# PaddlePaddle/PaddleRobotics

Measured on NVIDIA H100. Metric: env-steps/sec (A1, 4096 envs), higher is better.
Workload: dtype f32

## Files before the change

paddlerobotics_b200/csrc/b2q_math.cuh:

```cuda
#pragma once
#include <cmath>
#include <cstdint>

#if defined(__CUDACC__)
#define B2Q_HD __host__ __device__ __forceinline__
#define B2Q_D __device__ __forceinline__
#else
#define B2Q_HD inline
#define B2Q_D inline
#endif

namespace b2q {

B2Q_HD float m_sqrt(float x) { return sqrtf(x); }
B2Q_HD double m_sqrt(double x) { return sqrt(x); }
#if defined(__CUDA_ARCH__)
B2Q_HD float m_rsqrt(float x) { return rsqrtf(x); }
#else
B2Q_HD float m_rsqrt(float x) { return 1.0f / sqrtf(x); }
#endif
B2Q_HD double m_rsqrt(double x) { return 1.0 / sqrt(x); }
B2Q_HD float m_sin(float x) { return sinf(x); }
B2Q_HD double m_sin(double x) { return sin(x); }
B2Q_HD float m_cos(float x) { return cosf(x); }
// ... 15 lines not shown
B2Q_HD float m_min(float a, float b) { return fminf(a, b); }
B2Q_HD double m_min(double a, double b) { return fmin(a, b); }
B2Q_HD float m_max(float a, float b) { return fmaxf(a, b); }
B2Q_HD double m_max(double a, double b) { return fmax(a, b); }
B2Q_HD float m_fma(float a, float b, float c) { return fmaf(a, b, c); }
B2Q_HD double m_fma(double a, double b, double c) { return fma(a, b, c); }
B2Q_HD bool m_isfinite(float x) { return (x - x) == 0.0f; }
B2Q_HD bool m_isfinite(double x) { return (x - x) == 0.0; }
B2Q_HD bool m_isnan(float x) { return x != x; }
B2Q_HD bool m_isnan(double x) { return x != x; }

B2Q_HD float m_log(float x) { return logf(x); }
B2Q_HD double m_log(double x) { return log(x); }

B2Q_HD uint32_t mulhi32(uint32_t a, uint32_t b) { return (uint32_t)(((uint64_t)a * (uint64_t)b) >> 32); }
B2Q_HD void philox4(uint64_t seed, uint32_t c0, uint32_t c1, uint32_t c2, uint32_t out[4]) {
  uint32_t c3 = 0, k0 = (uint32_t)seed, k1 = (uint32_t)(seed >> 32);
  for (int i = 0; i < 10; i++) {
    uint32_t h0 = mulhi32(0xD2511F53u, c0), l0 = 0xD2511F53u * c0, h1 = mulhi32(0xCD9E8D57u, c2), l1 = 0xCD9E8D57u * c2;
    uint32_t n0 = h1 ^ c1 ^ k0, n2 = h0 ^ c3 ^ k1;
    c0 = n0; c1 = l1; c2 = n2; c3 = l0;
    k0 += 0x9E3779B9u; k1 += 0xBB67AE85u;
  }
  out[0] = c0; out[1] = c1; out[2] = c2; out[3] = c3;
}
template <typename T> B2Q_HD void philox_normal4(uint64_t seed, uint32_t c0, uint32_t c1, uint32_t c2, T n[4]) {
  uint32_t r[4]; philox4(seed, c0, c1, c2, r);
  const T two_pi = T(6.283185307179586476925286766559), sc = T(1.0 / 16777216.0);
  T u0 = (T(r[0] >> 8) + T(0.5)) * sc, u1 = (T(r[1] >> 8) + T(0.5)) * sc, u2 = (T(r[2] >> 8) + T(0.5)) * sc, u3 = (T(r[3] >> 8) + T(0.5)) * sc;
  T ra = m_sqrt(T(-2) * m_log(u0)), rb = m_sqrt(T(-2) * m_log(u2));
  n[0] = ra * m_cos(two_pi * u1); n[1] = ra * m_sin(two_pi * u1); n[2] = rb * m_cos(two_pi * u3); n[3] = rb * m_sin(two_pi * u3);
}

#if defined(__CUDA_ARCH__)
B2Q_HD float m_rcp(float x) { float r; asm("rcp.approx.ftz.f32 %0, %1;" : "=f"(r) : "f"(x)); return fmaf(r, fmaf(-x, r, 1.0f), r); }
#else
B2Q_HD float m_rcp(float x) { return 1.0f / x; }
#endif
B2Q_HD double m_rcp(double x) { return 1.0 / x; }

B2Q_HD void m_sincos(float a, float& s, float& c) {
  float q = rintf(a * 0.636619772367581343f);
  int n = (int)q;
  float r = fmaf(q, -1.57079601287841796875f, a);
  r = fmaf(q, -3.1391647326017846353352069854736328125e-7f, r);
  r = fmaf(q, -5.390302529957764765543e-15f, r);
  float r2 = r * r;
  float sp = fmaf(fmaf(fmaf(-1.95152959e-4f, r2, 8.33216087e-3f), r2, -1.66666546e-1f), r2 * r, r);
  float cp = fmaf(fmaf(fmaf(fmaf(2.44331571e-5f, r2, -1.38873163e-3f), r2, 4.16666457e-2f), r2, -0.5f), r2, 1.0f);
  float ss = (n & 1) ? cp : sp, cc = (n & 1) ? sp : cp;
  s = (n & 2) ? -ss : ss;
  c = ((n + 1) & 2) ? -cc : cc;
}
B2Q_HD void m_sincos(double a, double& s, double& c) { s = sin(a); c = cos(a); }

template <typename T>
struct V3 {
  T x, y, z;
};
template <typename T> B2Q_HD V3<T> mk(T x, T y, T z) { V3<T> r; r.x = x; r.y = y; r.z = z; return r; }
template <typename T> B2Q_HD V3<T> operator+(V3<T> a, V3<T> b) { return mk<T>(a.x + b.x, a.y + b.y, a.z + b.z); }
template <typename T> B2Q_HD V3<T> operator-(V3<T> a, V3<T> b) { return mk<T>(a.x - b.x, a.y - b.y, a.z - b.z); }
template <typename T> B2Q_HD V3<T> operator-(V3<T> a) { return mk<T>(-a.x, -a.y, -a.z); }
template <typename T> B2Q_HD V3<T> operator*(V3<T> a, T s) { return mk<T>(a.x * s, a.y * s, a.z * s); }
template <typename T> B2Q_HD V3<T> operator*(T s, V3<T> a) { return mk<T>(a.x * s, a.y * s, a.z * s); }
template <typename T> B2Q_HD T dot(V3<T> a, V3<T> b) { return a.x * b.x + a.y * b.y + a.z * b.z; }
// ... 1 lines not shown

template <typename T>
struct S3 {
  T xx, xy, xz, yy, yz, zz;
};
template <typename T> B2Q_HD V3<T> mul(const S3<T>& s, V3<T> v) {
  return mk<T>(s.xx * v.x + s.xy * v.y + s.xz * v.z, s.xy * v.x + s.yy * v.y + s.yz * v.z, s.xz * v.x + s.yz * v.y + s.zz * v.z);
}
template <typename T> B2Q_HD S3<T> operator+(const S3<T>& a, const S3<T>& b) { S3<T> r = {a.xx + b.xx, a.xy + b.xy, a.xz + b.xz, a.yy + b.yy, a.yz + b.yz, a.zz + b.zz}; return r; }
template <typename T> B2Q_HD S3<T> point_inertia(T m, V3<T> c) {
  S3<T> r = {m * (c.y * c.y + c.z * c.z), -m * c.x * c.y, -m * c.x * c.z, m * (c.x * c.x + c.z * c.z), -m * c.y * c.z, m * (c.x * c.x + c.y * c.y)};
  return r;
}

template <typename T>
struct R3 {
  V3<T> cx, cy, cz;
};
template <typename T> B2Q_HD V3<T> rot(const R3<T>& R, V3<T> v) { return R.cx * v.x + R.cy * v.y + R.cz * v.z; }
template <typename T> B2Q_HD V3<T> rotT(const R3<T>& R, V3<T> v) { return mk<T>(dot(R.cx, v), dot(R.cy, v), dot(R.cz, v)); }
template <typename T> B2Q_HD S3<T> rot_sym(const R3<T>& R, const S3<T>& I) {
  V3<T> a = R.cx * I.xx + R.cy * I.xy + R.cz * I.xz;
  V3<T> b = R.cx * I.xy + R.cy * I.yy + R.cz * I.yz;
  V3<T> c = R.cx * I.xz + R.cy * I.yz + R.cz * I.zz;
  S3<T> o;
  o.xx = a.x * R.cx.x + b.x * R.cy.x + c.x * R.cz.x;
  o.xy = a.x * R.cx.y + b.x * R.cy.y + c.x * R.cz.y;
  o.xz = a.x * R.cx.z + b.x * R.cy.z + c.x * R.cz.z;
  o.yy = a.y * R.cx.y + b.y * R.cy.y + c.y * R.cz.y;
  o.yz = a.y * R.cx.z + b.y * R.cy.z + c.y * R.cz.z;
  o.zz = a.z * R.cx.z + b.z * R.cy.z + c.z * R.cz.z;
  return o;
}
template <typename T> B2Q_HD R3<T> quat_to_R(T x, T y, T z, T w) {
  R3<T> R;
  R.cx = mk<T>(1 - 2 * (y * y + z * z), 2 * (x * y + z * w), 2 * (x * z - y * w));
  R.cy = mk<T>(2 * (x * y - z * w), 1 - 2 * (x * x + z * z), 2 * (y * z + x * w));
  R.cz = mk<T>(2 * (x * z + y * w), 2 * (y * z - x * w), 1 - 2 * (x * x + y * y));
  return R;
}
template <typename T> B2Q_HD V3<T> quat_to_rpy(T x, T y, T z, T w) {
  T s = 2 * (w * y - z * x);
  s = m_min(m_max(s, T(-1)), T(1));
  return mk<T>(m_atan2(2 * (w * x + y * z), 1 - 2 * (x * x + y * y)), m_asin(s), m_atan2(2 * (w * z + x * y), 1 - 2 * (y * y + z * z)));
}

template <typename T>
struct V6 {
  V3<T> a, l;
};
template <typename T> B2Q_HD V6<T> operator+(V6<T> p, V6<T> q) { V6<T> r; r.a = p.a + q.a; r.l = p.l + q.l; return r; }
template <typename T> B2Q_HD V6<T> operator-(V6<T> p, V6<T> q) { V6<T> r; r.a = p.a - q.a; r.l = p.l - q.l; return r; }
template <typename T> B2Q_HD V6<T> operator*(V6<T> p, T s) { V6<T> r; r.a = p.a * s; r.l = p.l * s; return r; }
template <typename T> B2Q_HD T dot6(V6<T> p, V6<T> q) { return dot(p.a, q.a) + dot(p.l, q.l); }
template <typename T> B2Q_HD T get6(const V6<T>& v, int i) { return i == 0 ? v.a.x : i == 1 ? v.a.y : i == 2 ? v.a.z : i == 3 ? v.l.x : i == 4 ? v.l.y : v.l.z; }

B2Q_HD constexpr int tri(int i, int j) { return i >= j ? i * (i + 1) / 2 + j : j * (j + 1) / 2 + i; }

template <typename T> B2Q_HD void chol6(T* S , T* Li ) {
#pragma unroll
  for (int j = 0; j < 6; j++) {
    T d = S[tri(j, j)];
#pragma unroll
    for (int k = 0; k < j; k++) d -= S[tri(j, k)] * S[tri(j, k)];
    T inv = m_rsqrt(d);
    S[tri(j, j)] = d * inv;
// ... 33 lines not shown
```

paddlerobotics_b200/csrc/b2q_sim.cuh:

```cuda
#pragma once
#include "b2q_math.cuh"

namespace b2q {

constexpr int NS = 37;
constexpr int NP = 15;
constexpr int NE = 16;
constexpr int OBS_DIM = 49;
constexpr int INFO_DIM = 56;
constexpr int ETG_H = 20;

template <typename T>
struct alignas(4 * sizeof(T)) P4 {
  T x, y, z, w;
};

template <typename T>
struct LegModel {
  T p1[3];
  T lhip;
  T com[3][3];
  T I[3][6];
  T m[3];
};
// ... 10 lines not shown
  T knee_r;
  int obs_dim, obs_identity;
  int obs_src[OBS_DIM];
  T obs_scale[OBS_DIM], obs_shift[OBS_DIM];
};
template <typename T>
struct Cfg {
  T dt; int R; int iters; T erp, warm, margin; int interp; T tau_limit; int settle_steps;
  int filter; T fb0, fb1, fb2, fa1, fa2; int etg; int max_steps;
  T etg_T, etg_T2, etg_sigma_sq, etg_amp, etg_ph0, etg_ph1;
  T w_torso, w_feet, w_up, w_tau, w_stand, w_badfoot, w_footcontact, w_done, reward_p, vel_d;
  int terrain, hf_nx, hf_ny; T hf_x0, hf_y0, hf_cell, hf_icell, idt; const T* hf;
  int clip_cmd; T max_dq;
  int noise_on; T noise[5]; unsigned long long noise_seed;
  int stuck, body_coll;
  int motor_mode, jlim, extf, knee; T damp[4];
};
constexpr int STUCK_H = 10;
template <typename T>
struct Buffers {
  int N, Dm;
  P4<T>* state;
  P4<T>* snap;
  P4<T>* snap_obs;
  const P4<T>* param;
  const P4<T>* etg;
  P4<T>* ring;
  int* step_count;
  P4<T>* pos_hist;
  const P4<T>* extf;
};
template <typename T>
struct LaneParam {
  T kp[3], kd[3], iscale[3], mscale[3], m0s, I0s[3], mu, latency;
  V3<T> g;
};
template <typename T>
struct LaneState {
  V3<T> pos; T qx, qy, qz, qw; V3<T> vlin, vang;
  T q[3], qd[3]; T lam_n; int contact;
  T lam_lim[3];
};

template <typename T> B2Q_HD void sincos_t(T a, T& s, T& c) { m_sincos(a, s, c); }

template <typename T>
B2Q_HD T terrain_height(const Cfg<T>& cf, T x, T y, V3<T>& n) {
  if (cf.terrain == 0) { n = mk<T>(0, 0, 1); return T(0); }
  T fx = (x - cf.hf_x0) * cf.hf_icell, fy = (y - cf.hf_y0) * cf.hf_icell;
  fx = m_min(m_max(fx, T(0)), T(cf.hf_nx) - T(1.000001));
  fy = m_min(m_max(fy, T(0)), T(cf.hf_ny) - T(1.000001));
  int ix = (int)fx, iy = (int)fy;
  if (ix > cf.hf_nx - 2) ix = cf.hf_nx - 2;
  if (iy > cf.hf_ny - 2) iy = cf.hf_ny - 2;
  T tx = fx - T(ix), ty = fy - T(iy);
  const T* h = cf.hf; int nx = cf.hf_nx;
  T h00 = h[iy * nx + ix], h10 = h[iy * nx + ix + 1], h01 = h[(iy + 1) * nx + ix], h11 = h[(iy + 1) * nx + ix + 1];
  T hh = (1 - tx) * (1 - ty) * h00 + tx * (1 - ty) * h10 + (1 - tx) * ty * h01 + tx * ty * h11;
  T dhdx = ((1 - ty) * (h10 - h00) + ty * (h11 - h01)) * cf.hf_icell;
  T dhdy = ((1 - tx) * (h01 - h00) + tx * (h11 - h10)) * cf.hf_icell;
  T inv = m_rsqrt(dhdx * dhdx + dhdy * dhdy + T(1));
  n = mk<T>(-dhdx * inv, -dhdy * inv, inv);
  return hh;
}

template <typename T>
struct LegKin {
// ... 110 lines not shown
    for (int i = 0; i < n; i++) {
      T ln = lam[i] + (vec[idx[i] * 4 + 1] - uu[i]) / W[i * NRW + i];
      if (par[i] >= 0) { T lim = mu * lam[par[i]]; ln = m_min(m_max(ln, -lim), lim); } else ln = m_max(ln, T(0));
      T dl = ln - lam[i]; lam[i] = ln;
      for (int j = 0; j < n; j++) uu[j] += W[j * NRW + i] * dl;
    }
  }
  for (int e = 0; e < RPL; e++) { const int q = pos_of[RPL * k + e]; lk[e] = q >= 0 ? lam[q] : T(0); }
  cm.sync();
}

template <typename T, int FEAT, class Comm>
B2Q_HD void substep(const Comm& cm, const Cfg<T>& cf, const Model<T>& md, const LaneParam<T>& pr, LaneState<T>& s,
                    const T* target, T* tau_out, V3<T> fext = V3<T>{0, 0, 0}, const T* hyb = nullptr ) {
  const int k = cm.leg();
  const LegModel<T>& lm = md.leg[k];
  const T dt = cf.dt, idt = cf.idt;
  R3<T> R = quat_to_R(s.qx, s.qy, s.qz, s.qw);
  V3<T> wB = rotT(R, s.vang), vB = rotT(R, s.vlin), gB = rotT(R, pr.g);

  T tau[3];
#pragma unroll
  for (int j = 0; j < 3; j++) {
    T cmd = target[j];
    if (cf.clip_cmd) cmd = m_min(m_max(cmd, s.q[j] - cf.max_dq), s.q[j] + cf.max_dq);
    T t = T(-1) * (pr.kp[j] * (s.q[j] - cmd)) - pr.kd[j] * (s.qd[j] - T(0));
    if (FEAT && cf.motor_mode == 1) t = target[j];
    if (FEAT && cf.motor_mode == 2) t = T(-1) * (hyb[j] * (s.q[j] - cmd)) - hyb[6 + j] * (s.qd[j] - hyb[3 + j]) + hyb[9 + j];
    if (cf.tau_limit > T(0)) t = m_min(m_max(t, -cf.tau_limit), cf.tau_limit);
    tau[j] = t; tau_out[j] = t;
  }

  LegKin<T> K; leg_kin(md, lm, s.q, K);
  const V3<T> a1 = mk<T>(1, 0, 0), a2 = K.a2;
  V3<T> cL[3]; S3<T> IL[3]; T mL[3];
  {
    const R3<T>* Rs[3] = {&K.R1, &K.R2, &K.R3m};
    const V3<T> ps[3] = {K.p1, K.p2, K.p3};
#pragma unroll
    for (int i = 0; i < 3; i++) {
      cL[i] = ps[i] + rot(*Rs[i], mk<T>(lm.com[i][0], lm.com[i][1], lm.com[i][2]));
      S3<T> Il = {lm.I[i][0], lm.I[i][1], lm.I[i][2], lm.I[i][3], lm.I[i][4], lm.I[i][5]};
      S3<T> Ib = rot_sym(*Rs[i], Il);
      T sc = pr.iscale[i];
      IL[i].xx = Ib.xx * sc; IL[i].xy = Ib.xy * sc; IL[i].xz = Ib.xz * sc; IL[i].yy = Ib.yy * sc; IL[i].yz = Ib.yz * sc; IL[i].zz = Ib.zz * sc;
      mL[i] = lm.m[i] * pr.mscale[i];
    }
  }
  V3<T> w1 = wB + a1 * s.qd[0], w2 = w1 + a2 * s.qd[1], w3 = w2 + a2 * s.qd[2];
  V3<T> pdd0 = cross(wB, vB) - gB;
  V3<T> al1 = cross(wB, a1) * s.qd[0];
  V3<T> pdd1 = pdd0 + cross(wB, cross(wB, K.p1));
  V3<T> al2 = al1 + cross(w1, a2) * s.qd[1];
  V3<T> d21 = K.p2 - K.p1;
  V3<T> pdd2 = pdd1 + cross(al1, d21) + cross(w1, cross(w1, d21));
  V3<T> al3 = al2 + cross(w2, a2) * s.qd[2];
  V3<T> d32 = K.p3 - K.p2;
  V3<T> pdd3 = pdd2 + cross(al2, d32) + cross(w2, cross(w2, d32));
  V3<T> fL[3], nL[3];
  {
    const V3<T> ws[3] = {w1, w2, w3}, als[3] = {al1, al2, al3}, pdds[3] = {pdd1, pdd2, pdd3}, ps[3] = {K.p1, K.p2, K.p3};
#pragma unroll
    for (int i = 0; i < 3; i++) {
      V3<T> r = cL[i] - ps[i];
      V3<T> cdd = pdds[i] + cross(als[i], r) + cross(ws[i], cross(ws[i], r));
      fL[i] = cdd * mL[i];
      nL[i] = mul(IL[i], als[i]) + cross(ws[i], mul(IL[i], ws[i]));
    }
  }
  V3<T> F3 = fL[2], N3 = nL[2] + cross(cL[2] - K.p3, fL[2]);
  V3<T> F2 = fL[1] + F3, N2 = nL[1] + cross(cL[1] - K.p2, fL[1]) + N3 + cross(d32, F3);
  V3<T> F1 = fL[0] + F2, N1 = nL[0] + cross(cL[0] - K.p1, fL[0]) + N2 + cross(d21, F2);
  T hj[3] = {dot(a1, N1), dot(a2, N2), dot(a2, N3)};
  V3<T> NO = N1 + cross(K.p1, F1);

  T m3c = mL[2], m2c = mL[1] + m3c, m1c = mL[0] + m2c;
  V3<T> h3c = cL[2] * mL[2], h2c = cL[1] * mL[1] + h3c, h1c = cL[0] * mL[0] + h2c;
  S3<T> I3c = IL[2] + point_inertia(mL[2], cL[2]);
  S3<T> I2c = IL[1] + point_inertia(mL[1], cL[1]) + I3c;
  S3<T> I1c = IL[0] + point_inertia(mL[0], cL[0]) + I2c;
  V3<T> v1 = cross(K.p1, a1), v2 = cross(K.p2, a2), v3 = cross(K.p3, a2);
  V6<T> Fc[3];
  Fc[0].a = mul(I1c, a1) + cross(h1c, v1); Fc[0].l = v1 * m1c + cross(a1, h1c);
  Fc[1].a = mul(I2c, a2) + cross(h2c, v2); Fc[1].l = v2 * m2c + cross(a2, h2c);
  Fc[2].a = mul(I3c, a2) + cross(h3c, v3); Fc[2].l = v3 * m3c + cross(a2, h3c);
  T M11 = dot(a1, Fc[0].a) + dot(v1, Fc[0].l);
  T M21 = dot(a1, Fc[1].a) + dot(v1, Fc[1].l), M22 = dot(a2, Fc[1].a) + dot(v2, Fc[1].l);
  T M31 = dot(a1, Fc[2].a) + dot(v1, Fc[2].l), M32 = dot(a2, Fc[2].a) + dot(v2, Fc[2].l), M33 = dot(a2, Fc[2].a) + dot(v3, Fc[2].l);
  T D[3][3];
  {
    T c00 = M22 * M33 - M32 * M32, c01 = M31 * M32 - M21 * M33, c02 = M21 * M32 - M31 * M22;
    T det = M11 * c00 + M21 * c01 + M31 * c02, id = m_rcp(det);
    D[0][0] = c00 * id; D[0][1] = D[1][0] = c01 * id; D[0][2] = D[2][0] = c02 * id;
    D[1][1] = (M11 * M33 - M31 * M31) * id; D[1][2] = D[2][1] = (M31 * M21 - M11 * M32) * id;
    D[2][2] = (M11 * M22 - M21 * M21) * id;
  }
  T bj[3] = {tau[0] - hj[0], tau[1] - hj[1], tau[2] - hj[2]};
  T Fa[3][6], FD[3][6];
#pragma unroll
  for (int i = 0; i < 3; i++) v6_to_arr(Fc[i], Fa[i]);
#pragma unroll
  for (int j = 0; j < 3; j++) {
#pragma unroll
    for (int c = 0; c < 6; c++) FD[j][c] = m_fma(Fa[2][c], D[2][j], m_fma(Fa[1][c], D[1][j], Fa[0][c] * D[0][j]));
  }

  T S[21], r6[6];
  {
    const T Z = T(0);
    const T Cf[6][6] = {{I1c.xx, I1c.xy, I1c.xz, Z, -h1c.z, h1c.y},
                        {I1c.xy, I1c.yy, I1c.yz, h1c.z, Z, -h1c.x},
                        {I1c.xz, I1c.yz, I1c.zz, -h1c.y, h1c.x, Z},
                        {Z, h1c.z, -h1c.y, m1c, Z, Z},
                        {-h1c.z, Z, h1c.x, Z, m1c, Z},
                        {h1c.y, -h1c.x, Z, Z, Z, m1c}};
#pragma unroll
    for (int i = 0; i < 6; i++) {
#pragma unroll
      for (int j = 0; j <= i; j++) {
        T v = Cf[i][j];
#pragma unroll
        for (int k = 0; k < 3; k++) v = m_fma(Fa[k][j], -FD[k][i], v);
        S[tri(i, j)] = cm.sum4(v);
      }
    }
    const T NOa[6] = {NO.x, NO.y, NO.z, F1.x, F1.y, F1.z};
#pragma unroll
    for (int i = 0; i < 6; i++) {
      T v = -NOa[i];
#pragma unroll
      for (int k = 0; k < 3; k++) v = m_fma(FD[k][i], -bj[k], v);
      r6[i] = cm.sum4(v);
    }
  }
  {
    T sx = m_sqrt(pr.I0s[0]), sy = m_sqrt(pr.I0s[1]), sz = m_sqrt(pr.I0s[2]);
    S3<T> I0 = {md.I0[0] * sx * sx, md.I0[1] * sx * sy, md.I0[2] * sx * sz, md.I0[3] * sy * sy, md.I0[4] * sy * sz, md.I0[5] * sz * sz};
    T m0 = md.m0 * pr.m0s;
    S[tri(0, 0)] += I0.xx; S[tri(1, 0)] += I0.xy; S[tri(1, 1)] += I0.yy; S[tri(2, 0)] += I0.xz; S[tri(2, 1)] += I0.yz; S[tri(2, 2)] += I0.zz;
    S[tri(3, 3)] += m0; S[tri(4, 4)] += m0; S[tri(5, 5)] += m0;
    V3<T> n0 = cross(wB, mul(I0, wB)), f0 = pdd0 * m0;
    if (FEAT) {
      T lv = m_sqrt(dot(vB, vB)), lw = m_sqrt(dot(wB, wB));
      f0 = f0 + vB * (m0 * (cf.damp[0] + cf.damp[1] * lv));
      n0 = n0 + mul(I0, wB) * (cf.damp[2] + cf.damp[3] * lw);
      if (cf.extf) f0 = f0 - rotT(R, fext);
    }
    r6[0] -= n0.x; r6[1] -= n0.y; r6[2] -= n0.z; r6[3] -= f0.x; r6[4] -= f0.y; r6[5] -= f0.z;
  }
  T Li[6];
  chol6(S, Li);
  fwd6(S, Li, r6); bwd6(S, Li, r6);
  V6<T> nud = arr_to_v6(r6);
  T qdd[3];
  {
    T t[3] = {bj[0] - dot6(Fc[0], nud), bj[1] - dot6(Fc[1], nud), bj[2] - dot6(Fc[2], nud)};
#pragma unroll
    for (int j = 0; j < 3; j++) qdd[j] = D[j][0] * t[0] + D[j][1] * t[1] + D[j][2] * t[2];
  }
  V3<T> wBs = wB + nud.a * dt, vBs = vB + (nud.l + cross(wB, vB)) * dt;
  T qds[3] = {s.qd[0] + dt * qdd[0], s.qd[1] + dt * qdd[1], s.qd[2] + dt * qdd[2]};

  V3<T> toe_w = s.pos + rot(R, K.toe), n_w;
  T hgt = terrain_height(cf, toe_w.x, toe_w.y, n_w);
  T dist = toe_w.z - hgt - md.foot_r;
  bool act = dist < cf.margin;
  V3<T> t1w = mk<T>(1 - n_w.x * n_w.x, -n_w.x * n_w.y, -n_w.x * n_w.z);
  t1w = t1w * m_rsqrt(dot(t1w, t1w));
  V3<T> t2w = cross(n_w, t1w);
  V3<T> eB[3] = {rotT(R, n_w), rotT(R, t1w), rotT(R, t2w)};
  V3<T> xc = K.toe - eB[0] * md.foot_r;
  T Jk[3][3], u[3], Y[3][6], Wl[3][3];
  {
    V3<T> r1 = cross(a1, xc - K.p1), r2 = cross(a2, xc - K.p2), r3 = cross(a2, xc - K.p3);
#pragma unroll
    for (int e = 0; e < 3; e++) {
      Jk[e][0] = dot(eB[e], r1); Jk[e][1] = dot(eB[e], r2); Jk[e][2] = dot(eB[e], r3);
      V6<T> Jb; Jb.a = cross(xc, eB[e]); Jb.l = eB[e];
      u[e] = dot(Jb.a, wBs) + dot(Jb.l, vBs) + Jk[e][0] * qds[0] + Jk[e][1] * qds[1] + Jk[e][2] * qds[2];
      const T Jba[6] = {Jb.a.x, Jb.a.y, Jb.a.z, Jb.l.x, Jb.l.y, Jb.l.z};
#pragma unroll
      for (int c = 0; c < 6; c++) {
        T g = Jba[c];
#pragma unroll
        for (int j = 0; j < 3; j++) g = m_fma(FD[j][c], -Jk[e][j], g);
        Y[e][c] = g;
      }
      fwd6(S, Li, Y[e]);
    }
#pragma unroll
    for (int e = 0; e < 3; e++) {
      T dj[3];
#pragma unroll
      for (int i = 0; i < 3; i++) dj[i] = D[i][0] * Jk[e][0] + D[i][1] * Jk[e][1] + D[i][2] * Jk[e][2];
#pragma unroll
      for (int e2 = 0; e2 < 3; e2++) Wl[e2][e] = Jk[e2][0] * dj[0] + Jk[e2][1] * dj[1] + Jk[e2][2] * dj[2];
    }
  }
  T lk[3] = {T(0), T(0), T(0)};
  T lkx[6] = {T(0), T(0), T(0), T(0), T(0), T(0)}, Yx[6][6], Jx[6][3];
#pragma unroll
  for (int e = 0; e < 6; e++) {
#pragma unroll
    for (int c = 0; c < 6; c++) Yx[e][c] = T(0);
    Jx[e][0] = Jx[e][1] = Jx[e][2] = T(0);
  }
  bool general = false;
  if constexpr (FEAT != 0) {
    bool need = false;
    T kdist = T(1); V3<T> kn_w = mk<T>(0, 0, 1);
    if (cf.jlim) {
#pragma unroll
      for (int j = 0; j < 3; j++) need = need || (s.q[j] - md.qlo[j] < JLIM_GAP) || (md.qhi[j] - s.q[j] < JLIM_GAP);
    }
    if (cf.knee) {
      V3<T> kw = s.pos + rot(R, K.p3);
      kdist = kw.z - terrain_height(cf, kw.x, kw.y, kn_w) - md.knee_r;
      need = need || (kdist < cf.margin);
    }
    if ((cf.jlim || cf.knee) && cm.any(need)) {
      T Y9[RPL][6], u9[RPL], targ9[RPL], warm9[RPL], blk[45], Jall[RPL][3]; bool act9[RPL];
#pragma unroll
      for (int e = 0; e < 3; e++) {
#pragma unroll
        for (int c = 0; c < 6; c++) Y9[e][c] = Y[e][c];
        u9[e] = u[e]; targ9[e] = T(0); warm9[e] = T(0); act9[e] = act;
        Jall[e][0] = Jk[e][0]; Jall[e][1] = Jk[e][1]; Jall[e][2] = Jk[e][2];
      }
      targ9[0] = dist > T(0) ? -dist * idt : cf.erp * (-dist) * idt; warm9[0] = cf.warm * s.lam_n;
      {
        const bool kact = cf.knee && (kdist < cf.margin);
        V3<T> t1k = mk<T>(1 - kn_w.x * kn_w.x, -kn_w.x * kn_w.y, -kn_w.x * kn_w.z);
        t1k = t1k * m_rsqrt(dot(t1k, t1k));
        V3<T> t2k = cross(kn_w, t1k);
        V3<T> ek[3] = {rotT(R, kn_w), rotT(R, t1k), rotT(R, t2k)};
        V3<T> xk = K.p3 - ek[0] * md.knee_r;
        V3<T> r1 = cross(a1, xk - K.p1), r2 = cross(a2, xk - K.p2), r3 = cross(a2, xk - K.p3);
#pragma unroll
        for (int e = 0; e < 3; e++) {
          T jr[3] = {dot(ek[e], r1), dot(ek[e], r2), dot(ek[e], r3)};
          V6<T> Jb; Jb.a = cross(xk, ek[e]); Jb.l = ek[e];
          u9[3 + e] = dot(Jb.a, wBs) + dot(Jb.l, vBs) + jr[0] * qds[0] + jr[1] * qds[1] + jr[2] * qds[2];
#pragma unroll
          for (int i = 0; i < 6; i++) Yx[e][i] = get6(Jb, i) - (FD[0][i] * jr[0] + FD[1][i] * jr[1] + FD[2][i] * jr[2]);
          fwd6(S, Li, Yx[e]);
          Jx[e][0] = jr[0]; Jx[e][1] = jr[1]; Jx[e][2] = jr[2];
          targ9[3 + e] = T(0); warm9[3 + e] = T(0); act9[3 + e] = kact;
        }
        targ9[3] = kdist > T(0) ? -kdist * idt : cf.erp * (-kdist) * idt;
      }
#pragma unroll
      for (int j = 0; j < 3; j++) {
        T glo = s.q[j] - md.qlo[j], ghi = md.qhi[j] - s.q[j], gap = glo, sj = T(1);
        if (ghi < glo) { gap = ghi; sj = T(-1); }
#pragma unroll
        for (int i = 0; i < 6; i++) Yx[3 + j][i] = -sj * FD[j][i];
        fwd6(S, Li, Yx[3 + j]);
        Jx[3 + j][0] = j == 0 ? sj : T(0); Jx[3 + j][1] = j == 1 ? sj : T(0); Jx[3 + j][2] = j == 2 ? sj : T(0);
        u9[6 + j] = sj * qds[j];
        targ9[6 + j] = gap > T(0) ? -gap * idt : cf.erp * (-gap) * idt;
        warm9[6 + j] = cf.warm * s.lam_lim[j];
        act9[6 + j] = cf.jlim && (gap < JLIM_GAP);
      }
#pragma unroll
      for (int e = 0; e < 6; e++) {
#pragma unroll
        for (int c = 0; c < 6; c++) Y9[3 + e][c] = Yx[e][c];
        Jall[3 + e][0] = Jx[e][0]; Jall[3 + e][1] = Jx[e][1]; Jall[3 + e][2] = Jx[e][2];
      }
#pragma unroll
// ... 138 lines not shown
    for (int i = 0; i < 3; i++) {
      jl[i] = Jk[0][i] * lk[0] + Jk[1][i] * lk[1] + Jk[2][i] * lk[2];
      if (FEAT != 0) jl[i] += Jx[0][i] * lkx[0] + Jx[1][i] * lkx[1] + Jx[2][i] * lkx[2] + Jx[3][i] * lkx[3] + Jx[4][i] * lkx[4] + Jx[5][i] * lkx[5];
      t[i] = jl[i] - dot6(Fc[i], dnu);
    }
#pragma unroll
    for (int j = 0; j < 3; j++) qds[j] += D[j][0] * t[0] + D[j][1] * t[1] + D[j][2] * t[2];
  }
  wBs = wBs + dnu.a; vBs = vBs + dnu.l;
  s.vang = rot(R, wBs); s.vlin = rot(R, vBs);
#pragma unroll
  for (int j = 0; j < 3; j++) { s.qd[j] = qds[j]; s.q[j] += dt * qds[j]; }
  s.pos = s.pos + s.vlin * dt;
  {
    T wx = s.vang.x, wy = s.vang.y, wz = s.vang.z, th = m_sqrt(wx * wx + wy * wy + wz * wz) * dt;
    T sh, cw; sincos_t(T(0.5) * th, sh, cw);
    T kk = th < T(1e-4) ? T(0.5) - th * th * T(1.0 / 48.0) : sh * m_rcp(th);
    T dx = wx * dt * kk, dy = wy * dt * kk, dz = wz * dt * kk;
    T ox = cw * s.qx + dx * s.qw + dy * s.qz - dz * s.qy;
    T oy = cw * s.qy - dx * s.qz + dy * s.qw + dz * s.qx;
    T oz = cw * s.qz + dx * s.qy - dy * s.qx + dz * s.qw;
    T ow = cw * s.qw - dx * s.qx - dy * s.qy - dz * s.qz;
    T nn = m_rsqrt(ox * ox + oy * oy + oz * oz + ow * ow);
    s.qx = ox * nn; s.qy = oy * nn; s.qz = oz * nn; s.qw = ow * nn;
  }
}

template <typename T> B2Q_HD P4<T> ldp(const P4<T>* base, int pack, int N, int env) { return base[(size_t)pack * N + env]; }
template <typename T> B2Q_HD void stp(P4<T>* base, int pack, int N, int env, T x, T y, T z, T w) {
  P4<T> p; p.x = x; p.y = y; p.z = z; p.w = w; base[(size_t)pack * N + env] = p;
}

template <typename T, class Comm>
B2Q_HD void load_param(const Comm& cm, const Buffers<T>& B, int env, LaneParam<T>& pr) {
  const int k = cm.leg(), N = B.N;
  P4<T> a = ldp(B.param, 0 + k, N, env), b = ldp(B.param, 4 + k, N, env), c = ldp(B.param, 8 + k, N, env);
  P4<T> d = ldp(B.param, 12, N, env), e = ldp(B.param, 13, N, env), g = ldp(B.param, 14, N, env);
  pr.kp[0] = a.x; pr.kp[1] = a.y; pr.kp[2] = a.z; pr.mu = a.w;
  pr.kd[0] = b.x; pr.kd[1] = b.y; pr.kd[2] = b.z; pr.latency = b.w;
  pr.iscale[0] = c.x; pr.iscale[1] = c.y; pr.iscale[2] = c.z;
  pr.mscale[0] = d.x; pr.mscale[1] = d.y; pr.mscale[2] = d.z; pr.m0s = d.w;
  pr.I0s[0] = e.x; pr.I0s[1] = e.y; pr.I0s[2] = e.z;
  pr.g = mk<T>(g.x, g.y, g.z);
}
template <typename T, class Comm>
B2Q_HD void load_state(const Comm& cm, const P4<T>* st, int N, int env, LaneState<T>& s, T* last_action, T* etg_act, int& has_last, V3<T>& rpy0) {
  const int k = cm.leg();
  P4<T> p0 = ldp(st, 0, N, env), p1 = ldp(st, 1, N, env), p2 = ldp(st, 2, N, env), p3 = ldp(st, 3, N, env);
  P4<T> pq = ldp(st, 4 + k, N, env), pd = ldp(st, 8 + k, N, env), pa = ldp(st, 12 + k, N, env), pe = ldp(st, 16 + k, N, env), pr = ldp(st, 20, N, env);
  s.pos = mk<T>(p0.x, p0.y, p0.z); s.qx = p1.x; s.qy = p1.y; s.qz = p1.z; s.qw = p1.w;
  s.vlin = mk<T>(p2.x, p2.y, p2.z); has_last = p2.w > T(0.5);
  s.vang = mk<T>(p3.x, p3.y, p3.z);
  s.q[0] = pq.x; s.q[1] = pq.y; s.q[2] = pq.z; s.lam_n = pq.w;
  s.qd[0] = pd.x; s.qd[1] = pd.y; s.qd[2] = pd.z; s.contact = pq.w > T(0);
  last_action[0] = pa.x; last_action[1] = pa.y; last_action[2] = pa.z; s.lam_lim[0] = pa.w; s.lam_lim[1] = pe.w; s.lam_lim[2] = pd.w;
  etg_act[0] = pe.x; etg_act[1] = pe.y; etg_act[2] = pe.z;
  rpy0 = mk<T>(pr.x, pr.y, pr.z);
}
template <typename T, class Comm>
B2Q_HD void store_state(const Comm& cm, P4<T>* st, int N, int env, const LaneState<T>& s, const T* last_action, const T* etg_act, int has_last, V3<T> rpy0) {
  const int k = cm.leg();
  if (k == 0) { stp(st, 0, N, env, s.pos.x, s.pos.y, s.pos.z, T(0)); stp(st, 20, N, env, rpy0.x, rpy0.y, rpy0.z, T(0)); }
  if (k == 1) stp(st, 1, N, env, s.qx, s.qy, s.qz, s.qw);
  if (k == 2) stp(st, 2, N, env, s.vlin.x, s.vlin.y, s.vlin.z, T(has_last));
  if (k == 3) stp(st, 3, N, env, s.vang.x, s.vang.y, s.vang.z, T(0));
  stp(st, 4 + k, N, env, s.q[0], s.q[1], s.q[2], s.lam_n);
  stp(st, 8 + k, N, env, s.qd[0], s.qd[1], s.qd[2], s.lam_lim[2]);
  stp(st, 12 + k, N, env, last_action[0], last_action[1], last_action[2], s.lam_lim[0]);
  stp(st, 16 + k, N, env, etg_act[0], etg_act[1], etg_act[2], s.lam_lim[1]);
}
template <typename T>
B2Q_HD void ring_write(const Buffers<T>& B, int slot, int ab, int k, int env, const T* q, const T* qd, const T* tau) {
  P4<T>* base = B.ring + ((size_t)(slot * 2 + ab) * 12) * B.N;
  stp(base, 3 * k + 0, B.N, env, q[0], q[1], q[2], tau[0]);
  stp(base, 3 * k + 1, B.N, env, qd[0], qd[1], qd[2], tau[1]);
// ... 40 lines not shown

template <typename T> B2Q_HD T obs_out_elem(const Model<T>& md, const T* full49, int j) {
  return md.obs_identity ? full49[j] : full49[md.obs_src[j]] * md.obs_scale[j] + md.obs_shift[j];
}

template <typename T, class Comm>
B2Q_HD void reset_lane(const Comm& cm, const Cfg<T>& cf, const Model<T>& md, const Buffers<T>& B, int env, bool valid, T* obs ,
                       const T* xoff = nullptr ) {
  const int k = cm.leg(), N = B.N;
  LaneState<T> s; T la[3], ea[3]; int hl; V3<T> rpy0;
  load_state(cm, B.snap, N, env, s, la, ea, hl, rpy0);
  T sq[3], sqd[3], stau[3];
  {
    P4<T> a = ldp(B.snap_obs, 3 * k, N, env), b = ldp(B.snap_obs, 3 * k + 1, N, env), c = ldp(B.snap_obs, 3 * k + 2, N, env);
    sq[0] = a.x; sq[1] = a.y; sq[2] = a.z; stau[0] = a.w; sqd[0] = b.x; sqd[1] = b.y; sqd[2] = b.z; stau[1] = b.w; stau[2] = c.x;
  }
  s.contact = s.lam_n > T(0);
  if (xoff) s.pos.x += xoff[env];
  rpy0 = quat_to_rpy(s.qx, s.qy, s.qz, s.qw);
  etg_act_leg(cm, cf, md, B.etg, N, env, T(0), ea);
  la[0] = la[1] = la[2] = T(0);
  if (valid) {
    store_state(cm, B.state, N, env, s, la, ea, 0, rpy0);
    for (int d = 0; d < B.Dm; d++) { ring_write(B, d, 0, k, env, sq, sqd, stau); ring_write(B, d, 1, k, env, sq, sqd, stau); }
    if (k == 0) B.step_count[env] = 0;
    if (cf.filter) for (int hslot = 0; hslot < 4; hslot++) stp(B.state, 21 + 4 * k + hslot, N, env, sq[0], sq[1], sq[2], T(0));
  }
  if (obs) write_obs(cm, md, obs, valid, s, s.pos, cf.dt * T(cf.R), rpy0, sq, sqd, ea);
}

template <typename T, int FEAT, class Comm>
B2Q_HD void settle_lane(const Comm& cm, const Cfg<T>& cf, const Model<T>& md, const Buffers<T>& B, int env, bool valid) {
  const int k = cm.leg(), N = B.N;
  LaneParam<T> pr; load_param(cm, B, env, pr);
  LaneState<T> s;
  s.pos = mk<T>(0, 0, T(0.32)); s.qx = s.qy = s.qz = 0; s.qw = 1; s.vlin = mk<T>(0, 0, 0); s.vang = mk<T>(0, 0, 0);
  T tgt[3], tau[3] = {0, 0, 0};
#pragma unroll
  for (int j = 0; j < 3; j++) { s.q[j] = md.pose_ori[j]; s.qd[j] = 0; tgt[j] = md.pose_ori[j]; }
  s.lam_n = 0; s.contact = 0; s.lam_lim[0] = s.lam_lim[1] = s.lam_lim[2] = 0;
  Cfg<T> cs = cf; cs.motor_mode = 0;
#pragma unroll 1
  for (int i = 0; i < cf.settle_steps; i++) substep<T, FEAT>(cm, cs, md, pr, s, tgt, tau);
  s.lam_lim[0] = s.lam_lim[1] = s.lam_lim[2] = T(0);
  if (valid) {
    T z3[3] = {0, 0, 0};
    store_state(cm, B.snap, N, env, s, z3, z3, 0, mk<T>(0, 0, 0));
    stp(B.snap_obs, 3 * k + 0, N, env, s.q[0], s.q[1], s.q[2], tau[0]);
    stp(B.snap_obs, 3 * k + 1, N, env, s.qd[0], s.qd[1], s.qd[2], tau[1]);
    stp(B.snap_obs, 3 * k + 2, N, env, tau[2], T(0), T(0), T(0));
  }
}

template <typename T, int FEAT, class Comm>
B2Q_HD void step_lane(const Comm& cm, const Cfg<T>& cf, const Model<T>& md, const Buffers<T>& B, int env, bool valid,
                      const T* action, int donef, int auto_reset, T* obs, T* reward, uint8_t* done, T* info, int obs_env0 = 0, int info_env0 = 0) {
  const int k = cm.leg(), N = B.N, R = cf.R;
  const T dtc = cf.dt * T(R);
  LaneParam<T> pr; load_param(cm, B, env, pr);
  LaneState<T> s; T last_action[3], etg_act[3]; int has_last; V3<T> rpy0;
  load_state(cm, B.state, N, env, s, last_action, etg_act, has_last, rpy0);
  int step = B.step_count[env];
  T target[3];
#pragma unroll
  for (int j = 0; j < 3; j++) target[j] = md.pose_ori[j] + etg_act[j] + action[(size_t)env * 12 + 3 * k + j];
  V3<T> fext = mk<T>(0, 0, 0);
  if (FEAT) {
    if (cf.motor_mode == 1) {
#pragma unroll
      for (int j = 0; j < 3; j++) target[j] = action[(size_t)env * 12 + 3 * k + j];
    }
    if (cf.extf) { P4<T> f = B.extf[env]; fext = mk<T>(f.x, f.y, f.z); }
  }
  T hyb[12] = {0, 0, 0, 0, 0, 0, 0, 0, 0, 0, 0, 0};
  if (FEAT && cf.motor_mode == 2) {
#pragma unroll
    for (int j = 0; j < 3; j++) {
      const T* a5 = action + ((size_t)env * 12 + 3 * k + j) * 5;
      target[j] = a5[0]; hyb[j] = a5[1]; hyb[3 + j] = a5[2]; hyb[6 + j] = a5[3]; hyb[9 + j] = a5[4];
    }
  }
  if (cf.filter && !(FEAT && cf.motor_mode == 2)) {
    P4<T> x1 = ldp(B.state, 21 + 4 * k, N, env), x2 = ldp(B.state, 22 + 4 * k, N, env), y1 = ldp(B.state, 23 + 4 * k, N, env), y2 = ldp(B.state, 24 + 4 * k, N, env);
    T ax1[3] = {x1.x, x1.y, x1.z}, ax2[3] = {x2.x, x2.y, x2.z}, ay1[3] = {y1.x, y1.y, y1.z}, ay2[3] = {y2.x, y2.y, y2.z}, yy[3];
#pragma unroll
    for (int j = 0; j < 3; j++) yy[j] = cf.fb0 * target[j] + cf.fb1 * ax1[j] + cf.fb2 * ax2[j] - cf.fa1 * ay1[j] - cf.fa2 * ay2[j];
    if (valid) {
      stp(B.state, 21 + 4 * k, N, env, target[0], target[1], target[2], T(0)); stp(B.state, 22 + 4 * k, N, env, ax1[0], ax1[1], ax1[2], T(0));
      stp(B.state, 23 + 4 * k, N, env, yy[0], yy[1], yy[2], T(0)); stp(B.state, 24 + 4 * k, N, env, ay1[0], ay1[1], ay1[2], T(0));
    }
#pragma unroll
    for (int j = 0; j < 3; j++) target[j] = yy[j];
  }
  const V3<T> start_pos = s.pos;
  T foot0_x;
  {
    LegKin<T> K; leg_kin(md, md.leg[k], s.q, K);
    R3<T> Rb = quat_to_R(s.qx, s.qy, s.qz, s.qw);
    foot0_x = s.pos.x + rot(Rb, K.toe).x;
  }
  int n_lag = pr.latency > T(0) ? (int)(pr.latency / cf.dt) : 0;
  T alpha = pr.latency > T(0) ? (pr.latency - T(n_lag) * cf.dt) / cf.dt : T(0);
  int max_lag = B.Dm * R - 2; if (n_lag > max_lag) { n_lag = max_lag; alpha = T(0); }
  int ia = ((R - 1 - n_lag) % R + R) % R, ma = (n_lag - (R - 1 - ia)) / R;
  int ib = ((R - 2 - n_lag) % R + R) % R, mb = (n_lag + 1 - (R - 1 - ib)) / R;
  const int slot = step % B.Dm;
  T tau[3] = {0, 0, 0};
#pragma unroll 1
  for (int i = 0; i < R; i++) {
    T proc[3];
    if (cf.interp && has_last && !(FEAT && cf.motor_mode == 2)) {
      T lerp = T(i + 1) / T(R);
#pragma unroll
      for (int j = 0; j < 3; j++) proc[j] = last_action[j] + lerp * (target[j] - last_action[j]);
    } else {
#pragma unroll
      for (int j = 0; j < 3; j++) proc[j] = target[j];
    }
    substep<T, FEAT>(cm, cf, md, pr, s, proc, tau, fext, hyb);
    if (valid && i == ia) ring_write(B, slot, 0, k, env, s.q, s.qd, tau);
    if (valid && i == ib) ring_write(B, slot, 1, k, env, s.q, s.qd, tau);
  }
#pragma unroll
  for (int j = 0; j < 3; j++) last_action[j] = target[j];
  has_last = 1;
  T dq[3], dqd[3], dtau[3];
  {
    T aq[3], aqd[3], at[3], bq[3], bqd[3], bt[3];
    ring_read(B, ((step - ma) % B.Dm + B.Dm) % B.Dm, 0, k, env, aq, aqd, at);
    ring_read(B, ((step - mb) % B.Dm + B.Dm) % B.Dm, 1, k, env, bq, bqd, bt);
#pragma unroll
    for (int j = 0; j < 3; j++) {
      dq[j] = (T(1) - alpha) * aq[j] + alpha * bq[j];
      dqd[j] = (T(1) - alpha) * aqd[j] + alpha * bqd[j];
      dtau[j] = (T(1) - alpha) * at[j] + alpha * bt[j];
    }
  }
  step += 1;
  T nz6[6] = {0, 0, 0, 0, 0, 0};
// ... 101 lines not shown
```

Before: 33.93 million.

## Specialize hip-axis math, hoist param-derived masses/inertia, prefetch ETG/snap buffers to L2

```diff
diff --git a/paddlerobotics_b200/csrc/b2q_math.cuh b/paddlerobotics_b200/csrc/b2q_math.cuh
--- a/paddlerobotics_b200/csrc/b2q_math.cuh
+++ b/paddlerobotics_b200/csrc/b2q_math.cuh
@@ -71,6 +71,14 @@
   n[0] = ra * m_cos(two_pi * u1); n[1] = ra * m_sin(two_pi * u1); n[2] = rb * m_cos(two_pi * u3); n[3] = rb * m_sin(two_pi * u3);
 }
 
+template <typename P> B2Q_HD void prefetch_l2(const P* p) {
+#if defined(__CUDA_ARCH__)
+  asm volatile("prefetch.global.L2 [%0];" ::"l"(p));
+#else
+  (void)p;
+#endif
+}
+
 #if defined(__CUDA_ARCH__)
 B2Q_HD float m_rcp(float x) { float r; asm("rcp.approx.ftz.f32 %0, %1;" : "=f"(r) : "f"(x)); return fmaf(r, fmaf(-x, r, 1.0f), r); }
 #else
@@ -138,6 +146,24 @@
   o.zz = a.z * R.cx.z + b.z * R.cy.z + c.z * R.cz.z;
   return o;
 }
+template <typename T> B2Q_HD V3<T> cross_ex(V3<T> p) { return mk<T>(T(0), p.z, -p.y); }
+template <typename T> B2Q_HD V3<T> ex_cross(V3<T> h) { return mk<T>(T(0), -h.z, h.y); }
+template <typename T> B2Q_HD T dot_0x(V3<T> v, V3<T> b) { return v.y * b.y + v.z * b.z; }
+template <typename T> B2Q_HD V3<T> cross_0x(V3<T> h, V3<T> v) { return mk<T>(h.y * v.z - h.z * v.y, -(h.x * v.z), h.x * v.y); }
+template <typename T> B2Q_HD V3<T> rot_ex(const R3<T>& R, V3<T> v) { return mk<T>(v.x, R.cy.y * v.y + R.cz.y * v.z, R.cy.z * v.y + R.cz.z * v.z); }
+template <typename T> B2Q_HD S3<T> rot_sym_ex(const R3<T>& R, const S3<T>& I) {
+  V3<T> a = mk<T>(I.xx, R.cy.y * I.xy + R.cz.y * I.xz, R.cy.z * I.xy + R.cz.z * I.xz);
+  V3<T> b = mk<T>(I.xy, R.cy.y * I.yy + R.cz.y * I.yz, R.cy.z * I.yy + R.cz.z * I.yz);
+  V3<T> c = mk<T>(I.xz, R.cy.y * I.yz + R.cz.y * I.zz, R.cy.z * I.yz + R.cz.z * I.zz);
+  S3<T> o;
+  o.xx = a.x;
+  o.xy = b.x * R.cy.y + c.x * R.cz.y;
+  o.xz = b.x * R.cy.z + c.x * R.cz.z;
+  o.yy = b.y * R.cy.y + c.y * R.cz.y;
+  o.yz = b.y * R.cy.z + c.y * R.cz.z;
+  o.zz = b.z * R.cy.z + c.z * R.cz.z;
+  return o;
+}
 template <typename T> B2Q_HD R3<T> quat_to_R(T x, T y, T z, T w) {
   R3<T> R;
   R.cx = mk<T>(1 - 2 * (y * y + z * z), 2 * (x * y + z * w), 2 * (x * z - y * w));
diff --git a/paddlerobotics_b200/csrc/b2q_sim.cuh b/paddlerobotics_b200/csrc/b2q_sim.cuh
--- a/paddlerobotics_b200/csrc/b2q_sim.cuh
+++ b/paddlerobotics_b200/csrc/b2q_sim.cuh
@@ -66,7 +66,8 @@
 };
 template <typename T>
 struct LaneParam {
-  T kp[3], kd[3], iscale[3], mscale[3], m0s, I0s[3], mu, latency;
+  T kp[3], kd[3], iscale[3], mu, latency;
+  T mL[3], m0; S3<T> I0;
   V3<T> g;
 };
 template <typename T>
@@ -243,24 +244,25 @@
   }
 
   LegKin<T> K; leg_kin(md, lm, s.q, K);
-  const V3<T> a1 = mk<T>(1, 0, 0), a2 = K.a2;
+  const V3<T> a2 = K.a2;
   V3<T> cL[3]; S3<T> IL[3]; T mL[3];
   {
     const R3<T>* Rs[3] = {&K.R1, &K.R2, &K.R3m};
     const V3<T> ps[3] = {K.p1, K.p2, K.p3};
 #pragma unroll
     for (int i = 0; i < 3; i++) {
-      cL[i] = ps[i] + rot(*Rs[i], mk<T>(lm.com[i][0], lm.com[i][1], lm.com[i][2]));
+      const V3<T> com = mk<T>(lm.com[i][0], lm.com[i][1], lm.com[i][2]);
+      cL[i] = ps[i] + (i == 0 ? rot_ex(K.R1, com) : rot(*Rs[i], com));
       S3<T> Il = {lm.I[i][0], lm.I[i][1], lm.I[i][2], lm.I[i][3], lm.I[i][4], lm.I[i][5]};
-      S3<T> Ib = rot_sym(*Rs[i], Il);
+      S3<T> Ib = i == 0 ? rot_sym_ex(K.R1, Il) : rot_sym(*Rs[i], Il);
       T sc = pr.iscale[i];
       IL[i].xx = Ib.xx * sc; IL[i].xy = Ib.xy * sc; IL[i].xz = Ib.xz * sc; IL[i].yy = Ib.yy * sc; IL[i].yz = Ib.yz * sc; IL[i].zz = Ib.zz * sc;
-      mL[i] = lm.m[i] * pr.mscale[i];
-    }
-  }
-  V3<T> w1 = wB + a1 * s.qd[0], w2 = w1 + a2 * s.qd[1], w3 = w2 + a2 * s.qd[2];
+      mL[i] = pr.mL[i];
+    }
+  }
+  V3<T> w1 = mk<T>(wB.x + s.qd[0], wB.y, wB.z), w2 = w1 + a2 * s.qd[1], w3 = w2 + a2 * s.qd[2];
   V3<T> pdd0 = cross(wB, vB) - gB;
-  V3<T> al1 = cross(wB, a1) * s.qd[0];
+  V3<T> al1 = mk<T>(T(0), wB.z * s.qd[0], -wB.y * s.qd[0]);
   V3<T> pdd1 = pdd0 + cross(wB, cross(wB, K.p1));
   V3<T> al2 = al1 + cross(w1, a2) * s.qd[1];
   V3<T> d21 = K.p2 - K.p1;
@@ -282,7 +284,7 @@
   V3<T> F3 = fL[2], N3 = nL[2] + cross(cL[2] - K.p3, fL[2]);
   V3<T> F2 = fL[1] + F3, N2 = nL[1] + cross(cL[1] - K.p2, fL[1]) + N3 + cross(d32, F3);
   V3<T> F1 = fL[0] + F2, N1 = nL[0] + cross(cL[0] - K.p1, fL[0]) + N2 + cross(d21, F2);
-  T hj[3] = {dot(a1, N1), dot(a2, N2), dot(a2, N3)};
+  T hj[3] = {N1.x, dot(a2, N2), dot(a2, N3)};
   V3<T> NO = N1 + cross(K.p1, F1);
 
   T m3c = mL[2], m2c = mL[1] + m3c, m1c = mL[0] + m2c;
@@ -290,14 +292,14 @@
   S3<T> I3c = IL[2] + point_inertia(mL[2], cL[2]);
   S3<T> I2c = IL[1] + point_inertia(mL[1], cL[1]) + I3c;
   S3<T> I1c = IL[0] + point_inertia(mL[0], cL[0]) + I2c;
-  V3<T> v1 = cross(K.p1, a1), v2 = cross(K.p2, a2), v3 = cross(K.p3, a2);
+  V3<T> v1 = cross_ex(K.p1), v2 = cross(K.p2, a2), v3 = cross(K.p3, a2);
   V6<T> Fc[3];
-  Fc[0].a = mul(I1c, a1) + cross(h1c, v1); Fc[0].l = v1 * m1c + cross(a1, h1c);
+  Fc[0].a = mk<T>(I1c.xx, I1c.xy, I1c.xz) + cross_0x(h1c, v1); Fc[0].l = mk<T>(T(0), v1.y * m1c - h1c.z, v1.z * m1c + h1c.y);
   Fc[1].a = mul(I2c, a2) + cross(h2c, v2); Fc[1].l = v2 * m2c + cross(a2, h2c);
   Fc[2].a = mul(I3c, a2) + cross(h3c, v3); Fc[2].l = v3 * m3c + cross(a2, h3c);
-  T M11 = dot(a1, Fc[0].a) + dot(v1, Fc[0].l);
-  T M21 = dot(a1, Fc[1].a) + dot(v1, Fc[1].l), M22 = dot(a2, Fc[1].a) + dot(v2, Fc[1].l);
-  T M31 = dot(a1, Fc[2].a) + dot(v1, Fc[2].l), M32 = dot(a2, Fc[2].a) + dot(v2, Fc[2].l), M33 = dot(a2, Fc[2].a) + dot(v3, Fc[2].l);
+  T M11 = Fc[0].a.x + dot_0x(v1, Fc[0].l);
+  T M21 = Fc[1].a.x + dot_0x(v1, Fc[1].l), M22 = dot(a2, Fc[1].a) + dot(v2, Fc[1].l);
+  T M31 = Fc[2].a.x + dot_0x(v1, Fc[2].l), M32 = dot(a2, Fc[2].a) + dot(v2, Fc[2].l), M33 = dot(a2, Fc[2].a) + dot(v3, Fc[2].l);
   T D[3][3];
   {
     T c00 = M22 * M33 - M32 * M32, c01 = M31 * M32 - M21 * M33, c02 = M21 * M32 - M31 * M22;
@@ -345,9 +347,8 @@
     }
   }
   {
-    T sx = m_sqrt(pr.I0s[0]), sy = m_sqrt(pr.I0s[1]), sz = m_sqrt(pr.I0s[2]);
-    S3<T> I0 = {md.I0[0] * sx * sx, md.I0[1] * sx * sy, md.I0[2] * sx * sz, md.I0[3] * sy * sy, md.I0[4] * sy * sz, md.I0[5] * sz * sz};
-    T m0 = md.m0 * pr.m0s;
+    const S3<T> I0 = pr.I0;
+    const T m0 = pr.m0;
     S[tri(0, 0)] += I0.xx; S[tri(1, 0)] += I0.xy; S[tri(1, 1)] += I0.yy; S[tri(2, 0)] += I0.xz; S[tri(2, 1)] += I0.yz; S[tri(2, 2)] += I0.zz;
     S[tri(3, 3)] += m0; S[tri(4, 4)] += m0; S[tri(5, 5)] += m0;
     V3<T> n0 = cross(wB, mul(I0, wB)), f0 = pdd0 * m0;
@@ -383,10 +384,10 @@
   V3<T> xc = K.toe - eB[0] * md.foot_r;
   T Jk[3][3], u[3], Y[3][6], Wl[3][3];
   {
-    V3<T> r1 = cross(a1, xc - K.p1), r2 = cross(a2, xc - K.p2), r3 = cross(a2, xc - K.p3);
+    V3<T> r1 = ex_cross(xc - K.p1), r2 = cross(a2, xc - K.p2), r3 = cross(a2, xc - K.p3);
 #pragma unroll
     for (int e = 0; e < 3; e++) {
-      Jk[e][0] = dot(eB[e], r1); Jk[e][1] = dot(eB[e], r2); Jk[e][2] = dot(eB[e], r3);
+      Jk[e][0] = dot_0x(r1, eB[e]); Jk[e][1] = dot(eB[e], r2); Jk[e][2] = dot(eB[e], r3);
       V6<T> Jb; Jb.a = cross(xc, eB[e]); Jb.l = eB[e];
       u[e] = dot(Jb.a, wBs) + dot(Jb.l, vBs) + Jk[e][0] * qds[0] + Jk[e][1] * qds[1] + Jk[e][2] * qds[2];
       const T Jba[6] = {Jb.a.x, Jb.a.y, Jb.a.z, Jb.l.x, Jb.l.y, Jb.l.z};
@@ -446,7 +447,7 @@
         V3<T> t2k = cross(kn_w, t1k);
         V3<T> ek[3] = {rotT(R, kn_w), rotT(R, t1k), rotT(R, t2k)};
         V3<T> xk = K.p3 - ek[0] * md.knee_r;
-        V3<T> r1 = cross(a1, xk - K.p1), r2 = cross(a2, xk - K.p2), r3 = cross(a2, xk - K.p3);
+        V3<T> r1 = ex_cross(xk - K.p1), r2 = cross(a2, xk - K.p2), r3 = cross(a2, xk - K.p3);
 #pragma unroll
         for (int e = 0; e < 3; e++) {
           T jr[3] = {dot(ek[e], r1), dot(ek[e], r2), dot(ek[e], r3)};
@@ -651,15 +652,19 @@
 }
 
 template <typename T, class Comm>
-B2Q_HD void load_param(const Comm& cm, const Buffers<T>& B, int env, LaneParam<T>& pr) {
+B2Q_HD void load_param(const Comm& cm, const Model<T>& md, const Buffers<T>& B, int env, LaneParam<T>& pr) {
   const int k = cm.leg(), N = B.N;
   P4<T> a = ldp(B.param, 0 + k, N, env), b = ldp(B.param, 4 + k, N, env), c = ldp(B.param, 8 + k, N, env);
   P4<T> d = ldp(B.param, 12, N, env), e = ldp(B.param, 13, N, env), g = ldp(B.param, 14, N, env);
   pr.kp[0] = a.x; pr.kp[1] = a.y; pr.kp[2] = a.z; pr.mu = a.w;
   pr.kd[0] = b.x; pr.kd[1] = b.y; pr.kd[2] = b.z; pr.latency = b.w;
   pr.iscale[0] = c.x; pr.iscale[1] = c.y; pr.iscale[2] = c.z;
-  pr.mscale[0] = d.x; pr.mscale[1] = d.y; pr.mscale[2] = d.z; pr.m0s = d.w;
-  pr.I0s[0] = e.x; pr.I0s[1] = e.y; pr.I0s[2] = e.z;
+  const T mscale[3] = {d.x, d.y, d.z};
+#pragma unroll
+  for (int i = 0; i < 3; i++) pr.mL[i] = md.leg[k].m[i] * mscale[i];
+  pr.m0 = md.m0 * d.w;
+  T sx = m_sqrt(e.x), sy = m_sqrt(e.y), sz = m_sqrt(e.z);
+  pr.I0 = {md.I0[0] * sx * sx, md.I0[1] * sx * sy, md.I0[2] * sx * sz, md.I0[3] * sy * sy, md.I0[4] * sy * sz, md.I0[5] * sz * sz};
   pr.g = mk<T>(g.x, g.y, g.z);
 }
 template <typename T, class Comm>
@@ -766,7 +771,7 @@
 template <typename T, int FEAT, class Comm>
 B2Q_HD void settle_lane(const Comm& cm, const Cfg<T>& cf, const Model<T>& md, const Buffers<T>& B, int env, bool valid) {
   const int k = cm.leg(), N = B.N;
-  LaneParam<T> pr; load_param(cm, B, env, pr);
+  LaneParam<T> pr; load_param(cm, md, B, env, pr);
   LaneState<T> s;
   s.pos = mk<T>(0, 0, T(0.32)); s.qx = s.qy = s.qz = 0; s.qw = 1; s.vlin = mk<T>(0, 0, 0); s.vang = mk<T>(0, 0, 0);
   T tgt[3], tau[3] = {0, 0, 0};
@@ -791,7 +796,7 @@
                       const T* action, int donef, int auto_reset, T* obs, T* reward, uint8_t* done, T* info, int obs_env0 = 0, int info_env0 = 0) {
   const int k = cm.leg(), N = B.N, R = cf.R;
   const T dtc = cf.dt * T(R);
-  LaneParam<T> pr; load_param(cm, B, env, pr);
+  LaneParam<T> pr; load_param(cm, md, B, env, pr);
   LaneState<T> s; T last_action[3], etg_act[3]; int has_last; V3<T> rpy0;
   load_state(cm, B.state, N, env, s, last_action, etg_act, has_last, rpy0);
   int step = B.step_count[env];
@@ -839,6 +844,14 @@
   int ia = ((R - 1 - n_lag) % R + R) % R, ma = (n_lag - (R - 1 - ia)) / R;
   int ib = ((R - 2 - n_lag) % R + R) % R, mb = (n_lag + 1 - (R - 1 - ib)) / R;
   const int slot = step % B.Dm;
+#pragma unroll
+  for (int p = k; p < NE; p += 4) prefetch_l2(B.etg + (size_t)p * N + env);
+  if (auto_reset) {
+#pragma unroll
+    for (int p = k; p < 21; p += 4) prefetch_l2(B.snap + (size_t)p * N + env);
+#pragma unroll
+    for (int p = k; p < 12; p += 4) prefetch_l2(B.snap_obs + (size_t)p * N + env);
+  }
   T tau[3] = {0, 0, 0};
 #pragma unroll 1
   for (int i = 0; i < R; i++) {
```

Result: faster. 34.59 million, median of 6 (+2.0%).
